# ami-iit/hippopt

Hardware: NVIDIA B200
Metric: knot_evals_per_s (higher is better)
Workload: dtype f64

## Files before the change

### hippopt_b200/_capi.py

```python
from __future__ import annotations

import ctypes
import os
import re

_HERE = os.path.dirname(os.path.abspath(__file__))
HEADER = os.path.join(os.path.dirname(_HERE), "include", "hippopt_b200.h")
LIB_PATH = os.environ.get("HIPPOPT_B200_LIB", os.path.join(_HERE, "libhippopt_b200.so"))


def parse_header(path: str = HEADER) -> dict[str, int]:
    text = open(path).read()
    text = re.sub(r"/\*.*?\*/", "", text, flags=re.S)
    text = re.sub(r"//[^\n]*", "", text)
    env: dict[str, int] = {}
    pattern = re.compile(r"#define\s+(\w+)\s+([^\n]+)|enum\s*\{([^}]*)\}", re.S)
    for mt in pattern.finditer(text):
        if mt.group(1):
            name, expr = mt.group(1), mt.group(2).strip()
            if not expr or name.endswith("_H"):
                continue
            try:
                env[name] = int(eval(expr, {"__builtins__": {}}, env))
            except Exception:
# ... 43 lines not shown
    L.hb_toy_create.argtypes = [ctypes.c_int32, ctypes.c_int32, ctypes.c_double, ctypes.POINTER(vp)]
    L.hb_destroy.restype = ctypes.c_int
    L.hb_destroy.argtypes = [vp]
    L.hb_dims.restype = ctypes.c_int
    L.hb_dims.argtypes = [vp, i64p, i64p, i64p, i64p, i64p]
    L.hb_pattern_jac.restype = ctypes.c_int
    L.hb_pattern_jac.argtypes = [vp, i64p, i64p]
    L.hb_pattern_hess.restype = ctypes.c_int
    L.hb_pattern_hess.argtypes = [vp, i64p, i64p]
    L.hb_eval.restype = ctypes.c_int
    L.hb_eval.argtypes = [vp, ctypes.c_uint32, vp, vp, ctypes.c_int64, vp, vp, vp, vp, vp, vp, vp, ctypes.c_int64, vp]
    L.hb_kino_attach_tables.restype = ctypes.c_int
    L.hb_kino_attach_tables.argtypes = [vp, i64p, i64p, i64p, i64p, i32p, f64p, i32p, f64p]
    L.hb_bounds.restype = ctypes.c_int
    L.hb_bounds.argtypes = [vp, f64p, f64p, f64p]
    L.hb_save.restype = ctypes.c_int
    L.hb_save.argtypes = [vp, ctypes.c_char_p]
    L.hb_load.restype = ctypes.c_int
    L.hb_load.argtypes = [ctypes.c_char_p, ctypes.POINTER(vp)]
    L.hb_ccs_group_mul.restype = ctypes.c_int
    L.hb_ccs_group_mul.argtypes = [vp, vp, vp, vp, vp, vp, vp, i64, i64, i64, i64, vp]
    L.hb_kkt_assemble_stage.restype = ctypes.c_int
    L.hb_kkt_assemble_stage.argtypes = [i32p, vp, vp, i64, vp, i64, vp, i64, vp, ctypes.c_double, vp, i64, vp, i64, vp, vp,
                                        vp, i64, vp]
    L.hb_external_bind.restype = ctypes.c_int
    L.hb_external_bind.argtypes = [vp]
    L.hb_external_stats.restype = ctypes.c_int
    L.hb_external_stats.argtypes = [i64p, i64p]
    L.hb_eval_cost_terms.restype = ctypes.c_int
    L.hb_eval_cost_terms.argtypes = [vp, vp, vp, ctypes.c_int64, vp, ctypes.c_int64, vp]
    L.hb_debug_sweep_schedule.restype = ctypes.c_int
    L.hb_debug_sweep_schedule.argtypes = [ctypes.c_int32, i32p, ctypes.c_int32, ctypes.c_int32, ctypes.c_int32,
                                          ctypes.c_int32, i32p, i32p]
    L.hb_host_set_parameters.restype = ctypes.c_int
    L.hb_host_set_parameters.argtypes = [vp, vp, ctypes.c_int64, ctypes.c_int64]
    L.hb_eval_host.restype = ctypes.c_int
    L.hb_eval_host.argtypes = [vp, ctypes.c_uint32, vp, vp, vp, vp, vp, vp, vp, vp, ctypes.c_int64]
    L.hb_host_last_traffic.restype = ctypes.c_int
    L.hb_host_last_traffic.argtypes = [vp, i64p, i64p]
    L.hb_host_alloc.restype = ctypes.c_int
    L.hb_host_alloc.argtypes = [ctypes.POINTER(vp), ctypes.c_int64]
    L.hb_host_free.restype = ctypes.c_int
    L.hb_host_free.argtypes = [vp]
    L.hb_lu_factor_batched.restype = ctypes.c_int
    L.hb_lu_factor_batched.argtypes = [vp, vp, vp, ctypes.c_int64, ctypes.c_int64, vp]
    L.hb_lu_solve_batched.restype = ctypes.c_int
    L.hb_lu_solve_batched.argtypes = [vp, vp, vp, ctypes.c_int64, ctypes.c_int64, ctypes.c_int64, vp]
    i64 = ctypes.c_int64
    L.hb_interpolate_humanoid_states.restype = ctypes.c_int
    L.hb_interpolate_humanoid_states.argtypes = [i64, i64, i64, vp, vp, vp, vp, i64, i64, vp, i64, i64, vp, vp, i64, i64, vp]
    L.hb_last_launch_count.restype = ctypes.c_int
    L.hb_last_launch_count.argtypes = [vp]
    L.hb_set_option.restype = ctypes.c_int
    L.hb_set_option.argtypes = [vp, ctypes.c_int32, ctypes.c_int32]
    L.hb_last_error.restype = ctypes.c_char_p
    L.hb_last_error.argtypes = []
    L.hb_profile_enable.restype = ctypes.c_int
    L.hb_profile_enable.argtypes = [vp, ctypes.c_int]
    L.hb_profile_read.restype = ctypes.c_int
    L.hb_profile_read.argtypes = [vp, f64p, i64p]
    L.hb_probe_fp64_tflops.restype = ctypes.c_int
    L.hb_probe_fp64_tflops.argtypes = [f64p, vp]
    _lib = L
    return L


EXPORTED_SYMBOLS = [
    "hb_kino_create", "hb_toy_create", "hb_destroy", "hb_dims", "hb_pattern_jac", "hb_pattern_hess", "hb_eval",
    "hb_last_launch_count", "hb_last_error", "hb_probe_fp64_tflops", "hb_profile_enable", "hb_profile_read",
    "hb_host_set_parameters", "hb_eval_host", "hb_host_last_traffic", "hb_host_alloc", "hb_host_free",
    "hb_lu_factor_batched", "hb_lu_solve_batched", "hb_set_option", "hb_interpolate_humanoid_states",
    "hb_eval_cost_terms", "hb_debug_sweep_schedule", "hb_kino_attach_tables", "hb_bounds", "hb_save", "hb_load",
    "hb_ccs_group_mul", "hb_external_bind", "hb_external_stats", "hb_kkt_assemble_stage",
] + ['hb_nlp_f', 'hb_nlp_f_n_in', 'hb_nlp_f_n_out', 'hb_nlp_f_sparsity_in', 'hb_nlp_f_sparsity_out', 'hb_nlp_f_work', 'hb_nlp_f_name_in', 'hb_nlp_f_name_out', 'hb_nlp_f_incref', 'hb_nlp_f_decref', 'hb_nlp_f_alloc_mem', 'hb_nlp_f_init_mem', 'hb_nlp_f_free_mem', 'hb_nlp_f_checkout', 'hb_nlp_f_release', 'hb_nlp_g', 'hb_nlp_g_n_in', 'hb_nlp_g_n_out', 'hb_nlp_g_sparsity_in', 'hb_nlp_g_sparsity_out', 'hb_nlp_g_work', 'hb_nlp_g_name_in', 'hb_nlp_g_name_out', 'hb_nlp_g_incref', 'hb_nlp_g_decref', 'hb_nlp_g_alloc_mem', 'hb_nlp_g_init_mem', 'hb_nlp_g_free_mem', 'hb_nlp_g_checkout', 'hb_nlp_g_release', 'hb_nlp_grad_f', 'hb_nlp_grad_f_n_in', 'hb_nlp_grad_f_n_out', 'hb_nlp_grad_f_sparsity_in', 'hb_nlp_grad_f_sparsity_out', 'hb_nlp_grad_f_work', 'hb_nlp_grad_f_name_in', 'hb_nlp_grad_f_name_out', 'hb_nlp_grad_f_incref', 'hb_nlp_grad_f_decref', 'hb_nlp_grad_f_alloc_mem', 'hb_nlp_grad_f_init_mem', 'hb_nlp_grad_f_free_mem', 'hb_nlp_grad_f_checkout', 'hb_nlp_grad_f_release', 'hb_nlp_jac_g', 'hb_nlp_jac_g_n_in', 'hb_nlp_jac_g_n_out', 'hb_nlp_jac_g_sparsity_in', 'hb_nlp_jac_g_sparsity_out', 'hb_nlp_jac_g_work', 'hb_nlp_jac_g_name_in', 'hb_nlp_jac_g_name_out', 'hb_nlp_jac_g_incref', 'hb_nlp_jac_g_decref', 'hb_nlp_jac_g_alloc_mem', 'hb_nlp_jac_g_init_mem', 'hb_nlp_jac_g_free_mem', 'hb_nlp_jac_g_checkout', 'hb_nlp_jac_g_release', 'hb_nlp_hess_l', 'hb_nlp_hess_l_n_in', 'hb_nlp_hess_l_n_out', 'hb_nlp_hess_l_sparsity_in', 'hb_nlp_hess_l_sparsity_out', 'hb_nlp_hess_l_work', 'hb_nlp_hess_l_name_in', 'hb_nlp_hess_l_name_out', 'hb_nlp_hess_l_incref', 'hb_nlp_hess_l_decref', 'hb_nlp_hess_l_alloc_mem', 'hb_nlp_hess_l_init_mem', 'hb_nlp_hess_l_free_mem', 'hb_nlp_hess_l_checkout', 'hb_nlp_hess_l_release']


class EvaluationError(RuntimeError):
    pass


def check(rc: int, what: str) -> None:
    if rc != 0:
        raise EvaluationError(f"{what} failed with code {rc}: {lib().hb_last_error().decode()}")
```

### hippopt_b200/csrc/api.cu

```cuda
#include <algorithm>
#include <cstdint>
#include <cstdio>
#include <cstring>
#include <map>
#include <string>
#include <vector>

#include "kino_const.cuh"
#include "contact_jac_desc.h"


static thread_local std::string g_err;
static int fail(int code, const std::string& msg) {
  g_err = msg;
  return code;
}
#define CUDA_TRY(expr)                                                                      \
  do {                                                                                      \
    cudaError_t e__ = (expr);                                                               \
    if (e__ != cudaSuccess) return fail(HB_ERR_CUDA, std::string(#expr) + ": " + cudaGetErrorString(e__)); \
  } while (0)

enum { KIND_KINO = 1, KIND_TOY = 2 };

// ... 78 lines not shown
  if ((e = cudaFuncSetAttribute(hb::lu_factor_kernel<3, 1>, cudaFuncAttributeMaxDynamicSharedMemorySize, lu_big)) != cudaSuccess) return e;
  if ((e = cudaFuncSetAttribute(hb::lu_factor_kernel<1, 2>, cudaFuncAttributeMaxDynamicSharedMemorySize, lu_big)) != cudaSuccess) return e;
  if ((e = cudaFuncSetAttribute(hb::lu_factor_kernel<2, 2>, cudaFuncAttributeMaxDynamicSharedMemorySize, lu_big)) != cudaSuccess) return e;
  if ((e = cudaFuncSetAttribute(hb::lu_solve_kernel, cudaFuncAttributeMaxDynamicSharedMemorySize, lu_big)) != cudaSuccess) return e;
  const int lu_staged = 232448 - 1024 - 2560;
  if ((e = cudaFuncSetAttribute(hb::lu_solve_staged_kernel<4>, cudaFuncAttributeMaxDynamicSharedMemorySize, lu_staged)) != cudaSuccess) return e;
  if ((e = cudaFuncSetAttribute(hb::lu_solve_staged_kernel<3>, cudaFuncAttributeMaxDynamicSharedMemorySize, lu_staged)) != cudaSuccess) return e;
  if ((e = cudaFuncSetAttribute(hb::lu_solve_staged_kernel<2>, cudaFuncAttributeMaxDynamicSharedMemorySize, lu_staged)) != cudaSuccess) return e;
  if ((e = cudaFuncSetAttribute(hb::lu_solve_staged_kernel<1>, cudaFuncAttributeMaxDynamicSharedMemorySize, lu_staged)) != cudaSuccess) return e;
  if ((e = cudaDeviceGetAttribute(&device_sms[dev], cudaDevAttrMultiProcessorCount, dev)) != cudaSuccess) return e;
  done[dev] = true;
  return cudaSuccess;
}

__global__ void reduce_f_kernel(const double* __restrict__ fpart, double* __restrict__ f, int n_terms, long batch) {
  const long b = (long)blockIdx.x * blockDim.x + threadIdx.x;
  if (b >= batch) return;
  const double* fp = fpart + b * n_terms;
  double acc = 0.0;
  for (int i = 0; i < n_terms; ++i) acc += fp[i];
  f[b] = acc;
}

static hb::SweepTopo sweep_topo_of(const hb::KinoConst& C) {
  hb::SweepTopo T;
  T.nb = C.nb;
  for (int l = 0; l < 32; ++l) {
    T.parent[l] = l < C.nb ? C.body[l].parent : -1;
    T.sub_mask[l] = C.sub_mask[l];
  }
  T.foot_body[0] = C.foot_body[0];
  T.foot_body[1] = C.foot_body[1];
  T.chest_body = C.chest_body;
  return T;
}

extern "C" int hb_debug_sweep_schedule(int32_t nb, const int32_t* parent, int32_t foot_l, int32_t foot_r, int32_t chest,
                                       int32_t typed, int32_t* tasks, int32_t* info) {
  if (!parent || !tasks || !info || nb < 2 || nb > 28) return fail(HB_ERR_INVALID, "hb_debug_sweep_schedule: bad argument");
  hb::SweepTopo T;
  T.nb = nb;
  for (int l = 0; l < 32; ++l) {
    T.parent[l] = l < nb ? parent[l] : -1;
    T.sub_mask[l] = 0u;
  }
  for (int l = 0; l < nb; ++l)
    for (int b = l; b >= 0; b = T.parent[b]) T.sub_mask[b] |= 1u << l;
  T.foot_body[0] = foot_l;
  T.foot_body[1] = foot_r;
  T.chest_body = chest;
  const hb::SweepSchedule s = hb::build_sweep_schedule(T, typed != 0, typed >= 2 ? 0 : 1);
  if (s.n_rounds <= 0) return fail(HB_ERR_UNSUPPORTED, "hb_debug_sweep_schedule: no schedule");
  for (size_t i = 0; i < s.tasks.size() && i < 32 * 32; ++i) tasks[i] = s.tasks[i];
  info[0] = s.n_rounds;
  info[1] = s.n_slots;
  info[2] = s.n_tasks;
  info[3] = s.n_heavy_tasks;
  info[4] = (int32_t)s.heavy_mask;
  info[5] = (int32_t)s.seed_mask;
  for (int d = 0; d < 27 && d < 4 + nb - 1; ++d) info[6 + d] = s.root_slot[d];
  return HB_OK;
}

template <class T>
static cudaError_t upload(T** dst, const T* src, size_t n) {
  cudaError_t e = cudaMalloc(dst, n * sizeof(T) + 16);
  if (e != cudaSuccess) return e;
  return cudaMemcpy(*dst, src, n * sizeof(T), cudaMemcpyHostToDevice);
}

extern "C" int hb_kino_create(const int32_t* icfg, const double* dcfg, const int32_t* jc_map, const int32_t* jk_map,
                              const int16_t* hc_index, const int32_t* hc_map, const int32_t* hk_map,
                              const int32_t* hk2_map, hb_handle* out) {
  if (!icfg || !dcfg || !jc_map || !jk_map || !hc_index || !hc_map || !hk_map || !hk2_map || !out)
    return fail(HB_ERR_INVALID, "hb_kino_create: null argument");
  hb_problem_s* h = new hb_problem_s();
  h->kind = KIND_KINO;
  cudaGetDevice(&h->device);
  hb::KinoConst& C = h->host;
  C.N = icfg[HB_KI_HORIZON];
  C.n_x = icfg[HB_KI_N_X];
  C.n_p = icfg[HB_KI_N_P];
  C.m = icfg[HB_KI_M];
  C.nnz_j = icfg[HB_KI_NNZ_J];
  C.nnz_h = icfg[HB_KI_NNZ_H];
  C.n_jc = icfg[HB_KI_N_JC];
  C.n_jk = icfg[HB_KI_N_JK];
  C.n_hc = icfg[HB_KI_N_HC];
  C.terrain = icfg[HB_KI_TERRAIN];
  C.has_final = icfg[HB_KI_HAS_FINAL];
  C.has_per = icfg[HB_KI_HAS_PERIODICITY];
  C.h_init = icfg[HB_KI_H_INIT];
  C.po_desc0 = icfg[HB_KI_PO_DESC0];
  C.po_mass = icfg[HB_KI_PO_MASS];
// ... 1354 lines not shown
```

### hippopt_b200/csrc/kino_kin.cu

```cuda
#include "kino_const.cuh"

namespace hb {

enum {
  SB_O = 0, SB_D = 3, SB_W = 6, SB_V = 9, SB_AX = 12, SB_I = 15, SB_R = 21, SB_L = 30, SB_IH = 33, SB_RHO = 36,
  SB_ACC = 39, SB_STRIDE = 51,
  SB_CB = SB_R, SB_CDB = SB_R + 3
};
enum { HSTAGE = 27 * 57 };
#ifndef HB_KIN_STAGE
#define HB_KIN_STAGE 1
#endif
#ifndef HB_KIN_STAGE_F
#define HB_KIN_STAGE_F 0
#endif
#ifndef HB_FWD_JAC
#define HB_FWD_JAC 1
#endif
#if HB_FWD_JAC && !HB_KIN_STAGE
#error "HB_FWD_JAC stages the Jacobian columns: it needs HB_KIN_STAGE"
#endif
#ifndef KIN_SCAT
#define KIN_SCAT 17
#endif
// ... 371 lines not shown
    emit.joint_t(l, dot(tax, np) + dot(ax, cn), dot(tax, wp) + dot(ax, cw));
    const int p = C.parent[l];
    const D3 rho = ld3(bl + SB_RHO), wpar = ld3(sb + p * SB_STRIDE + SB_W);
    const double inp = ((dir.mask >> p) & 1u) ? 1.0 : 0.0;
    const D3 ap = scale(inp, dir.alpha);
    const D3 trho = cross(ap, rho);
    const D3 twpar = cross(ap, wpar - dir.wpi) + scale(inp, dir.u);
    const double sd = zs[Z_SD + l - 1];
    const D3 pn = cn + cross(trho, Fp) + cross(rho, cF) + scale(sd, cross(tax, wp) + cross(ax, cw)) +
                  cross(trho, cross(vp, wpar)) + cross(rho, cross(cv, wpar) + cross(vp, twpar));
    const D3 pw = cw + cross(trho, vp) + cross(rho, cv);
    if (p == l - 1) {
      cn = pn;
      cw = pw;
    } else if (p == 0) {
      An = An + pn;
      AF = AF + cF;
      Aw = Aw + pw;
      Av = Av + cv;
    } else {
      double* sl = slot + C.slot[p] * 12 * 32 + lane;
      slot_add(sl, 0, pn);
      slot_add(sl, 3, cF);
      slot_add(sl, 6, pw);
      slot_add(sl, 9, cv);
    }
  }
  n0 = cn;
  w0 = cw;
  v0 = cv;
}

struct DirData {
  D3 alpha, pi, wpi, vpi, u;
};
__device__ __forceinline__ D3 shfl3(const D3& v, int src) {
  return v3<double>(__shfl_sync(0xffffffffu, v.x, src), __shfl_sync(0xffffffffu, v.y, src),
                    __shfl_sync(0xffffffffu, v.z, src));
}

__device__ __forceinline__ void kin_tangent_sweep_packed(const KinTopo& T, const double* sb, const double* zs,
                                                         const double* qdat, const double* massv, const SeedsT& ownS,
                                                         D3 hb, double* pslot, double* stage) {
  const int lane = threadIdx.x & 31;
  const D3 zero = v3<double>(0.0, 0.0, 0.0);
  for (int i = lane; i < T.n_pslots * 12; i += 32) pslot[i] = 0.0;
  __syncwarp();
  D3 cn = zero, cF = zero, cw = zero, cv = zero;
  unsigned t_next = (unsigned)T.sched[lane];
  for (int r = 0; r < T.n_rounds; ++r) {
    const unsigned t = t_next;
    if (r + 1 < T.n_rounds) t_next = (unsigned)T.sched[(r + 1) * 32 + lane];
    const bool valid = (t & KT_VALID) != 0;
    const int l = (t >> KT_L_SHIFT) & 31, p = (t >> KT_P_SHIFT) & 31, d = (t >> KT_D_SHIFT) & 31;
    const int src = valid ? d : lane;
    const bool heavy = (T.round_heavy_mask >> r) & 1u;
    SeedsT S;
    S.footF[0] = S.footF[1] = S.footN[0] = S.footN[1] = S.chestN = zero;
    if ((T.round_seed_mask >> r) & 1u) {
      S.footF[0] = shfl3(ownS.footF[0], src);
      S.footF[1] = shfl3(ownS.footF[1], src);
      S.footN[0] = shfl3(ownS.footN[0], src);
      S.footN[1] = shfl3(ownS.footN[1], src);
      S.chestN = shfl3(ownS.chestN, src);
    }
    if (valid) {
      if (t & KT_START) cn = cF = cw = cv = zero;
      const double* bl = sb + l * SB_STRIDE;
      const D3 ax = ld3(bl + SB_AX);
      D3 tax = zero, trho = zero, twpar = zero;
      const D3 rho = ld3(bl + SB_RHO), wpar = ld3(sb + p * SB_STRIDE + SB_W);
      if (heavy) {
        DirData dir;
        {
          const double* bd = sb + (d < 4 ? 0 : d - 3) * SB_STRIDE;
          dir.wpi = ld3(bd + SB_W);
          dir.vpi = ld3(bd + SB_V);
          if (d < 4) {
            dir.alpha = ld3(qdat + 6 * d);
            dir.u = ld3(qdat + 6 * d + 3);
            dir.pi = zero;
          } else {
            dir.alpha = ld3(bd + SB_AX);
            dir.u = zero;
            dir.pi = ld3(bd + SB_O);
          }
        }
        const double m = massv[l];
        const bool in = (t & KT_IN_L) != 0;
        const D3 a = in ? dir.alpha : zero, uu = in ? dir.u : zero;
        const D3 d_ = ld3(bl + SB_D), w = ld3(bl + SB_W);
        const D3 rr = ld3(bl + SB_O) - dir.pi;
        const D3 to = cross(a, rr);
        const D3 td = cross(a, d_);
        const D3 tw = cadd(uu, a, w - dir.wpi);
        const D3 tv = cadd(cadd(cross(dir.wpi, to), a, (ld3(bl + SB_V) - dir.vpi) - cross(dir.wpi, rr)), uu, rr);
        tax = cross(a, ax);
        if (in) {
          const double* I = bl + SB_I;
          const D3 cbar = ld3(bl + SB_CB), cdbar = ld3(bl + SB_CDB), Ih = ld3(bl + SB_IH), Iw = ld3(bl + SB_L);
          const D3 tc = to + td;
          const D3 tcd = cadd(cadd(tv, tw, d_), w, td);
          const D3 tcbar = scale(m, cross(tcd, hb));
          const D3 tcdbar = scale(m, cross(hb, tc));
          const D3 tIw = cadd(symmul(I, tw - cross(a, w)), a, Iw);
          const D3 tIh = csub(cross(a, Ih), I, cross(a, hb));
          cF = cF + tcbar;
          D3 n1 = cadd(cadd(cadd(cn, td, cbar), d_, tcbar), td, cross(cdbar, w));
          D3 n2 = cadd(cadd(cadd(cross(d_, cadd(cross(tcdbar, w), cdbar, tw)), tIw, hb), tIh, w), Ih, tw);
          cn = n1 + n2;
          cv = cv + tcdbar;
          cw = cadd(cadd(cw, td, cdbar), d_, tcdbar) + tIh;
        }
        if (t & KT_IN_P) {
          trho = cross(dir.alpha, rho);
          twpar = cadd(dir.u, dir.alpha, wpar - dir.wpi);
        }
      }
      if (l == T.foot_body[0]) {
        cF = cF + S.footF[0];
        cn = cn + S.footN[0];
      }
      if (l == T.foot_body[1]) {
        cF = cF + S.footF[1];
        cn = cn + S.footN[1];
      }
      if (l == T.chest_body) cn = cn + S.chestN;
      const int ls = (t >> KT_LOAD_SHIFT) & 63;
      if (ls) {
        const double* sl = pslot + (ls - 1) * 12;
        cn = cn + ld3(sl);
        cF = cF + ld3(sl + 3);
        cw = cw + ld3(sl + 6);
        cv = cv + ld3(sl + 9);
      }
      if (l != 0) {
        double* col = stage + d * 57;
        const double sd = zs[Z_SD + l - 1];
        if (heavy) {
          const D3 np = ld3(bl + SB_ACC), Fp = ld3(bl + SB_ACC + 3), wp = ld3(bl + SB_ACC + 6), vp = ld3(bl + SB_ACC + 9);
          col[7 + l - 1] += dot(tax, wp) + dot(ax, cw);
          col[34 + l - 1] += dot(tax, np) + dot(ax, cn);
          D3 n1 = cadd(cadd(cn, trho, Fp), rho, cF);
          D3 n2 = cadd(scale(sd, cadd(cross(tax, wp), ax, cw)), trho, cross(vp, wpar));
          cn = cadd(n1 + n2, rho, cadd(cross(cv, wpar), vp, twpar));
          cw = cadd(cadd(cw, trho, vp), rho, cv);
        } else {
          col[7 + l - 1] += dot(ax, cw);
          col[34 + l - 1] += dot(ax, cn);
// ... 574 lines not shown
        unsigned w[8];
#pragma unroll
        for (int u = 0; u < 8; ++u) w[u] = (eb + 32 * u) < n ? lst[eb + 32 * u] : 0xffffffffu;
#pragma unroll
        for (int u = 0; u < 8; ++u)
          if (w[u] != 0xffffffffu) em.jac[w[u] & 0xffffu] = st[w[u] >> 16];
      }
      __syncwarp();
    }
    if (want_grad) {
      double* gf = grad_f + b * T.n_x + (long)k * T.x_stride;
      for (int i = lane; i < 57; i += 32) {
        int off;
        if (i < 3) off = Z_VB + i;
        else if (i < 7) off = Z_QD + i - 3;
        else if (i < 11) off = Z_Q + i - 7;
        else if (i < 34) off = Z_SD + i - 11;
        else off = Z_S + i - 34;
        if (C.zmap[off] >= 0) gf[C.zmap[off]] = gbuf[i];
      }
      if (lane < 3 && C.zmap[Z_PB + lane] >= 0) gf[C.zmap[Z_PB + lane]] = 0.0;
    }
  }
  if (!WITH_HESS) return;
  if (!with_l && !(HB_FWD_JAC && (want_jac || want_grad))) return;
  {
    const int dirj = lane < 27 ? lane : -1;
    Dir dir;
    dir.mask = 0u;
    dir.alpha = dir.pi = dir.wpi = dir.vpi = dir.u = v3<double>(0.0, 0.0, 0.0);
    double* qdat = zs;
    double* qw = zs + 48;
    double* qK = zs + 60;
    static_assert(48 + 12 + 32 <= Z_VB && HB_N_JOINTS + 1 <= 24, "quaternion tables overlap z or the masses");
    if (lane < 4) {
      D3 g, u, w;
      const double qraw[4] = {q0, q1, q2, q3};
      quat_map<double>(qraw, qdv, lane, g, u, w);
      st3(qdat + 6 * lane, g);
      st3(qdat + 6 * lane + 3, u);
      st3(qw + 3 * lane, w);
    }
    __syncwarp();
    D3 wq_lane = v3<double>(0.0, 0.0, 0.0);
    if (lane >= 3 && lane < 7) wq_lane = ld3(qw + 3 * (lane - 3));
    if (lane < 4) {
      dir.alpha = ld3(qdat + 6 * lane);
      dir.u = ld3(qdat + 6 * lane + 3);
      dir.mask = 0xffffffffu;
      dir.wpi = ld3(sb + SB_W);
      dir.vpi = ld3(sb + SB_V);
    } else if (lane < 27) {
      const int l = lane - 4 + 1;
      dir.mask = C.sub_mask[l];
      const double* bl = sb + l * SB_STRIDE;
      dir.alpha = ld3(bl + SB_AX);
      dir.pi = ld3(bl + SB_O);
      dir.wpi = ld3(bl + SB_W);
      dir.vpi = ld3(bl + SB_V);
    }
    enum { CM_M = 0, CM_P = 1, CM_PD = 4, CM_H = 7, CM_J = 10, CM_STRIDE = 17 };
    double* comp = sm + L.stage;
    if (lane < nb) {
      const double* bl = sb + lane * SB_STRIDE;
      const double m = my_mass;
      const D3 c = ld3(bl + SB_O) + ld3(bl + SB_D);
      const D3 cd = ld3(bl + SB_V) + cross(ld3(bl + SB_W), ld3(bl + SB_D));
// ... 43 lines not shown
    }
    HB_PHASE(0, 4);
    D3 tP, tPd, th;
    {
      const double* cm = comp + (lane >= 4 && lane < 27 ? lane - 3 : 0) * CM_STRIDE;
      const double Ms = cm[CM_M];
      const D3 P = ld3(cm + CM_P), Pds = ld3(cm + CM_PD), Hs = ld3(cm + CM_H);
      const D3 a = dir.alpha, beta = cross(dir.alpha, dir.wpi);
      const D3 Pr = P - scale(Ms, dir.pi);
      tP = cross(a, Pr);
      tPd = cross(a, Pds - scale(Ms, dir.vpi)) - cross(beta, Pr) + cross(dir.u, P);
      th = cross(a, Hs) - cross(cross(a, dir.pi), Pds) - cross(P, cross(a, dir.vpi)) - symmul(cm + CM_J, beta) +
           cross(P, cross(beta, dir.pi)) + symmul(cm + CM_J, dir.u);
    }
    D3 vel_dh = v3<double>(0.0, 0.0, 0.0);
    D3 vel_pv = vel_dh;
    if (lane < 30) {
      D3 A = v3<double>(0.0, 0.0, 0.0), B = A, piv = A;
      int lv = 0;
      if (lane < 3) B = v3<double>(lane == 0 ? 1.0 : 0.0, lane == 1 ? 1.0 : 0.0, lane == 2 ? 1.0 : 0.0);
      else if (lane < 7) A = wq_lane;
      else {
        lv = lane - 6;
        A = ld3(sb + lv * SB_STRIDE + SB_AX);
        piv = ld3(sb + lv * SB_STRIDE + SB_O);
      }
      const double* cm = comp + lv * CM_STRIDE;
      const double Ms = cm[CM_M];
      const D3 P = ld3(cm + CM_P);
      const D3 pv = cross(A, P - scale(Ms, piv)) + scale(Ms, B);
      const D3 hv = symmul(cm + CM_J, A) - cross(P, cross(A, piv)) + cross(P, B);
      vel_dh = scale(-1.0 / mass_p, hv - scale(1.0 / M, cross(Pm, pv)));
      vel_pv = pv;
    }
    __syncwarp();
    const V3<Dual> xcD = lift<Dual>(xc, scale(1.0 / M, tP));
    const V3<Dual> xdD = lift<Dual>(xcd, scale(1.0 / M, tPd));
    const double inL = ((dir.mask >> T.foot_body[0]) & 1u) ? 1.0 : 0.0;
    const double inR = ((dir.mask >> T.foot_body[1]) & 1u) ? 1.0 : 0.0;
    const double inC = ((dir.mask >> T.chest_body) & 1u) ? 1.0 : 0.0;
    double ty_lane, tphi_lane;
    {
      const D3 a = dir.alpha;
      const D3 tL = scale(inL, cross(a, (ld3(sb + T.foot_body[0] * SB_STRIDE + SB_O) - dir.pi) + fdal));
      const D3 tR = scale(inR, cross(a, (ld3(sb + T.foot_body[1] * SB_STRIDE + SB_O) - dir.pi) + fdar));
      ty_lane = dot(scale(inR, cross(a, fdu)), fdDelta) + dot(fdu, tL - tR);
      const D3 ac = scale(inC, a);
      tphi_lane = cross(ac, v3<double>(G[0], G[3], G[6])).x + cross(ac, v3<double>(G[1], G[4], G[7])).y +
                  cross(ac, v3<double>(G[2], G[5], G[8])).z;
    }
    HB_PHASE(0, 5);
#if HB_FWD_JAC
    if (want_jac || want_grad) {
      double* stg = sm + L.stage;
      const int bm = 4 + 648 + 81;
      if (want_jac) {
        if (lane < 27) {
#pragma unroll
          for (int pt = 0; pt < 8; ++pt) {
            const int f = pt >> 2;
            const double in = f == 0 ? inL : inR;
            const D3 r = (ld3(sb + T.foot_body[f] * SB_STRIDE + SB_O) - dir.pi) + ld3(sm + L.arms + 3 * pt);
            const D3 t = scale(-in, cross(dir.alpha, r));
            stg[4 + (3 * pt) * 27 + lane] = t.x;
            stg[4 + (3 * pt + 1) * 27 + lane] = t.y;
            stg[4 + (3 * pt + 2) * 27 + lane] = t.z;
// ... 98 lines not shown
      S.footF[1] = S.footF[1] - ku;
      S.footN[1] = S.footN[1] + scale(kd, cross(uD, dD)) - cross(arD, ku);
    }
    {
      const D3 a = scale(inC, dir.alpha);
      double tG[9];
#pragma unroll
      for (int j = 0; j < 3; ++j) {
        const D3 col = v3<double>(G[j], G[3 + j], G[6 + j]);
        const D3 t = cross(a, col);
        tG[j] = t.x;
        tG[3 + j] = t.y;
        tG[6 + j] = t.z;
      }
      const double tphi = tG[0] + tG[4] + tG[8];
      const double cw = k1 ? 2.0 * sg * T.w_frame : 0.0;
      const Dual kappa = mkdual(cw * (phi - 3.0), cw * tphi);
      const V3<Dual> mGD = lift<Dual>(mG, v3<double>(tG[5] - tG[7], tG[6] - tG[2], tG[1] - tG[3]));
      S.chestN = scale(kappa, mGD);
    }
    HessEmit em;
    em.map = C.hk_map + T.knot_maps[k].hk_off;
    em.hess = hess + b * T.nnz_h + T.knot_maps[k].hk_base;
    em.stage = HB_KIN_STAGE ? sm + L.stage : nullptr;
    em.dirj = dirj;
    em.add_sd = em.add_s = 0.0;
    if (lane >= 4 && lane < 27 && k1) {
      const double wjl = C.wj[lane - 4];
      em.add_sd = T.joint_cost_kind == 0 ? sg * T.w_joint * 2.0 * wjl : 0.0;
      em.add_s = T.joint_cost_kind == 0 ? sg * T.w_joint * 2.0 * wjl * wjl : sg * T.w_joint * 2.0 * wjl;
    }
    V3<Dual> n0, w0, v0;
    const double lu_pre = lamk[31];
#ifdef HB_DUAL_SWEEP
    kin_backward<Dual>(T, sb, zs, dir, S, xcD, xdD, slot, em, n0, w0, v0);
#else
    {
      SeedsP SP;
      SeedsT ST;
      SP.wc = S.wc;
      SP.hb = S.hb;
#pragma unroll
      for (int f = 0; f < 2; ++f) {
        SP.footF[f] = primal_of(S.footF[f]);
        SP.footN[f] = primal_of(S.footN[f]);
        ST.footF[f] = tangent_of(S.footF[f]);
        ST.footN[f] = tangent_of(S.footN[f]);
      }
      SP.chestN = primal_of(S.chestN);
      ST.chestN = tangent_of(S.chestN);
      __syncwarp();
      HB_PHASE(0, 8);
      primal_adjoint_pass(T, sb, zs, SP, xc, xcd, my_depth, my_rank, my_parent, my_mass);
      HB_PHASE(0, 9);
      D3 tn0, tw0, tv0;
#if HB_SWEEP_PACKED
      {
        double* stg = sm + L.stage;
        double* pslot = sm + L.gbuf;
        constexpr int XT = 7;
        double* xt = pslot;
        double* massv = zs + 24;
        if (lane < 27) {
          st3(xt + (30 + lane) * XT, tP);
          st3(xt + (30 + lane) * XT + 3, tPd);
        }
        if (lane < 30) st3(xt + lane * XT + 3, vel_pv);
        if (lane < nb) massv[lane] = my_mass;
        __syncwarp();
        if (lane < 27) {
          const D3 hbv = S.hb;
          const D3 a1 = cross(tPd, hbv), a2 = cross(hbv, tP);
          double* col = stg + lane * 57;
          const double sM = -1.0 / M;
#pragma unroll 5
          for (int r = 0; r < 30; ++r) col[r] = sM * dot(ld3(xt + XT * r + 3), a2);
#pragma unroll 2
          for (int j = 0; j < 14; ++j) {
            const int e = lane + j < 27 ? lane + j : lane + j - 27;
            const double* xe = xt + XT * (30 + e);
            const double v = sM * (dot(ld3(xe), a1) + dot(ld3(xe + 3), a2));
            col[30 + e] = v;
            stg[e * 57 + 30 + lane] = v;
          }
          if (lane >= 4) {
            col[7 + lane - 4] += em.add_sd;
            col[34 + lane - 4] += em.add_s;
          }
        }
        __syncwarp();
        HB_PHASE(0, 10);
        em.acc = true;
        kin_tangent_sweep_packed(T, sb, zs, qdat, massv, ST, S.hb, pslot, stg);
        HB_PHASE(0, 11);
        const double* rs = pslot + (lane < 27 ? T.root_slot[lane] : 0) * 12;
        tn0 = ld3(rs);
        tw0 = ld3(rs + 6);
        tv0 = ld3(rs + 9);
      }
#else
      kin_tangent_sweep(T, sb, zs, dir, S.hb, ST, tangent_of(xcD), tangent_of(xdD), slot, em, tn0, tw0, tv0);
#endif
      n0 = lift<Dual>(ld3(sb + SB_ACC), tn0);
      w0 = lift<Dual>(ld3(sb + SB_ACC + 6), tw0);
      v0 = lift<Dual>(ld3(sb + SB_ACC + 9), tv0);
    }
#endif
    if (lane < 16) {
      const int a = lane >> 2, bq = lane & 3;
      Dual qD[4];
      double qdv2[4];
#pragma unroll
      for (int i = 0; i < 4; ++i) {
        qD[i] = mkdual(zs[Z_Q + i], i == bq ? 1.0 : 0.0);
        qdv2[i] = zs[Z_QD + i];
      }
      V3<Dual> g, u, w;
      quat_map<Dual>(qD, qdv2, a, g, u, w);
      const D3 pn0 = primal_of(n0), pw0 = primal_of(w0);
      qK[lane] = dot(pn0, tangent_of(g)) + dot(pw0, tangent_of(u));
      qK[16 + lane] = dot(pw0, tangent_of(w));
    }
    __syncwarp();
    if (dirj >= 0) {
      const D3 tn0 = tangent_of(n0), tw0 = tangent_of(w0);
      em.put(0, v0.x.d);
      em.put(1, v0.y.d);
      em.put(2, v0.z.d);
      const double lu = lu_pre;
      const double nqd = rbq[0] * rbq[0] + rbq[1] * rbq[1] + rbq[2] * rbq[2] +
                         rbq[3] * rbq[3];
#pragma unroll
      for (int a = 0; a < 4; ++a) {
        const bool qdir = lane < 4;
        const double dq = dot(tn0, ld3(qdat + 6 * a)) + dot(tw0, ld3(qdat + 6 * a + 3)) + (qdir ? qK[4 * a + lane] : 0.0);
        const double dqd = dot(tw0, ld3(qw + 3 * a)) + (qdir ? qK[16 + 4 * a + lane] : 0.0);
        const double extra = (a == lane && k1) ? 2.0 * sg * T.w_bq * nqd + 2.0 * lu : 0.0;
        em.put(3 + a, dqd);
        em.put(30 + a, dq + extra);
      }
    }
    HB_PHASE(0, 12);
    __syncwarp();
    if (em.stage) {
      const double* st = sm + L.stage;
#if HB_KIN_HESS_LIST
      const int2 hkl = *reinterpret_cast<const int2*>(&T.knot_maps[k].hk_off);
      const unsigned* lst = C.hk_list + hkl.x;
      const int n = hkl.y;
      for (int eb = lane; eb < n; eb += 32 * KIN_SCAT) {
        unsigned w[KIN_SCAT];
#pragma unroll
        for (int u = 0; u < KIN_SCAT; ++u) w[u] = (eb + 32 * u) < n ? lst[eb + 32 * u] : 0xffffffffu;
#pragma unroll
        for (int u = 0; u < KIN_SCAT; ++u)
          if (w[u] != 0xffffffffu) em.hess[w[u] & 0xffffu] = st[w[u] >> 16];
      }
#else
      for (int eb = lane; eb < HSTAGE; eb += 32 * KIN_SCAT) {
        int sl[KIN_SCAT];
#pragma unroll
        for (int u = 0; u < KIN_SCAT; ++u) sl[u] = (eb + 32 * u) < HSTAGE ? em.map[eb + 32 * u] : -1;
#pragma unroll
        for (int u = 0; u < KIN_SCAT; ++u)
          if (sl[u] >= 0) em.hess[sl[u]] = st[eb + 32 * u];
      }
#endif
    }
    if (lane < 27) {
      const int2 hk2m = *reinterpret_cast<const int2*>(&T.knot_maps[k].hk2_base);
      const int slot2 = C.hk2_map[hk2m.y + lane];
      if (slot2 >= 0)
// ... 15 lines not shown
```

### hippopt_b200/csrc/sweep_schedule.h

```cpp
#pragma once
#include <algorithm>
#include <map>
#include <utility>
#include <vector>

namespace hb {

enum {
  KT_L_SHIFT = 0, KT_P_SHIFT = 5, KT_D_SHIFT = 10, KT_VALID = 1 << 15, KT_START = 1 << 16, KT_IN_L = 1 << 17,
  KT_IN_P = 1 << 18, KT_LOAD_SHIFT = 19, KT_FLUSH_SHIFT = 25, KT_STORE = 1u << 31
};

struct SweepTopo {
  int nb = 0;
  int parent[32];
  int foot_body[2];
  int chest_body = 0;
  unsigned sub_mask[32];
};

struct SweepSchedule {
  std::vector<int> tasks;
  int n_rounds = 0, n_slots = 0, n_tasks = 0, n_heavy_tasks = 0;
  unsigned seed_mask = 0;
  unsigned heavy_mask = 0;
  int root_slot[32] = {0};
};

inline SweepSchedule build_sweep_schedule(const SweepTopo& C, bool typed_rounds = true, int policy = 1) {
  const int nb = C.nb, n_dir = 4 + (nb - 1);
  struct Seg {
    int d;
    std::vector<int> bodies;
    int flush_body;
    int crit = 0, lane = -1, next = 0, flushed = -1;
    std::vector<int> round_of;
  };
  std::vector<Seg> segs;
  std::vector<std::vector<int>> slot_of(n_dir, std::vector<int>(nb, -1));
  std::vector<std::vector<char>> in_full(n_dir, std::vector<char>(nb, 0));
  int n_slots = 0;
  for (int d = 0; d < n_dir; ++d) {
    const int ld = d < 4 ? 0 : d - 3;
    std::vector<char> rel(nb, 0);
    for (int l = 0; l < nb; ++l)
      if ((C.sub_mask[ld] >> l) & 1u) in_full[d][l] = rel[l] = 1;
    for (int a = C.parent[ld]; a >= 0; a = C.parent[a]) rel[a] = 1;
    for (int f = 0; f < 2; ++f)
      if (in_full[d][C.foot_body[f]])
        for (int a = C.foot_body[1 - f]; a >= 0; a = C.parent[a]) rel[a] = 1;
    std::vector<int> height(nb, 0), main_child(nb, -1);
    for (int l = nb - 1; l >= 1; --l) {
      if (!rel[l]) continue;
      const int p = C.parent[l];
      if (rel[p] && height[l] + 1 > height[p]) {
        height[p] = height[l] + 1;
        main_child[p] = l;
      }
    }
    slot_of[d][0] = n_slots++;
    for (int l = nb - 1; l >= 1; --l) {
      if (!rel[l]) continue;
      bool leaf = true;
      for (int c = l + 1; c < nb; ++c)
        if (rel[c] && C.parent[c] == l) leaf = false;
      if (!leaf) continue;
      Seg s;
      s.d = d;
      int b = l;
      for (;;) {
        s.bodies.push_back(b);
        const int p = C.parent[b];
        if (p == 0 || main_child[p] != b) {
          s.flush_body = p;
          break;
// ... 148 lines not shown
```

### include/hippopt_b200.h

```cpp
#ifndef HIPPOPT_B200_H
#define HIPPOPT_B200_H

#include <stdint.h>

#ifdef __cplusplus
extern "C" {
#endif

typedef struct hb_problem_s* hb_handle;

enum {
  HB_EVAL_F = 1,
  HB_EVAL_GRAD_F = 2,
  HB_EVAL_G = 4,
  HB_EVAL_JAC_G = 8,
  HB_EVAL_HESS_L = 16
};

enum { HB_OK = 0, HB_ERR_INVALID = 1, HB_ERR_CUDA = 2, HB_ERR_UNSUPPORTED = 3 };

#define HB_MAX_BODIES 32
#define HB_N_JOINTS 23
#define HB_N_POINTS 8

// ... 245 lines not shown
int hb_nlp_jac_g(const double** arg, double** res, hb_casadi_int* iw, double* w, int mem);
hb_casadi_int hb_nlp_jac_g_n_in(void);
hb_casadi_int hb_nlp_jac_g_n_out(void);
const hb_casadi_int* hb_nlp_jac_g_sparsity_in(hb_casadi_int i);
const hb_casadi_int* hb_nlp_jac_g_sparsity_out(hb_casadi_int i);
int hb_nlp_jac_g_work(hb_casadi_int* sz_arg, hb_casadi_int* sz_res, hb_casadi_int* sz_iw, hb_casadi_int* sz_w);
const char* hb_nlp_jac_g_name_in(hb_casadi_int i);
const char* hb_nlp_jac_g_name_out(hb_casadi_int i);
void hb_nlp_jac_g_incref(void);
void hb_nlp_jac_g_decref(void);
int hb_nlp_jac_g_alloc_mem(void);
int hb_nlp_jac_g_init_mem(int mem);
void hb_nlp_jac_g_free_mem(int mem);
int hb_nlp_jac_g_checkout(void);
void hb_nlp_jac_g_release(int mem);
int hb_nlp_hess_l(const double** arg, double** res, hb_casadi_int* iw, double* w, int mem);
hb_casadi_int hb_nlp_hess_l_n_in(void);
hb_casadi_int hb_nlp_hess_l_n_out(void);
const hb_casadi_int* hb_nlp_hess_l_sparsity_in(hb_casadi_int i);
const hb_casadi_int* hb_nlp_hess_l_sparsity_out(hb_casadi_int i);
int hb_nlp_hess_l_work(hb_casadi_int* sz_arg, hb_casadi_int* sz_res, hb_casadi_int* sz_iw, hb_casadi_int* sz_w);
const char* hb_nlp_hess_l_name_in(hb_casadi_int i);
const char* hb_nlp_hess_l_name_out(hb_casadi_int i);
void hb_nlp_hess_l_incref(void);
void hb_nlp_hess_l_decref(void);
int hb_nlp_hess_l_alloc_mem(void);
int hb_nlp_hess_l_init_mem(int mem);
void hb_nlp_hess_l_free_mem(int mem);
int hb_nlp_hess_l_checkout(void);
void hb_nlp_hess_l_release(int mem);

int hb_debug_sweep_schedule(int32_t nb, const int32_t* parent, int32_t foot_l, int32_t foot_r, int32_t chest,
                            int32_t typed, int32_t* tasks, int32_t* info);

const char* hb_last_error(void);

int hb_probe_fp64_tflops(double* tflops, void* stream);

#ifdef __cplusplus
}
#endif
#endif
```

Measured before the change: 22.70 million.

## Compute base-orientation tangent directions in closed form instead of through the packed sweep

Removes the four base-quaternion directions from the packed tangent sweep schedule (n_base=0 in the device topology) and computes their root tangent contributions analytically in lanes 0-3, storing them in a new shared table. Stage columns are patched to add the missing terms via lam_al and vel_dh rows. This shortens the sweep schedule (fewer tasks and rounds) at the cost of extra closed-form arithmetic and more complex correctness reasoning. The debug schedule API gains an n_base variant that keeps the old default of 4.

```diff
diff --git a/hippopt_b200/_capi.py b/hippopt_b200/_capi.py
--- a/hippopt_b200/_capi.py
+++ b/hippopt_b200/_capi.py
@@ -99,6 +99,9 @@
     L.hb_debug_sweep_schedule.restype = ctypes.c_int
     L.hb_debug_sweep_schedule.argtypes = [ctypes.c_int32, i32p, ctypes.c_int32, ctypes.c_int32, ctypes.c_int32,
                                           ctypes.c_int32, i32p, i32p]
+    L.hb_debug_sweep_schedule_n_base.restype = ctypes.c_int
+    L.hb_debug_sweep_schedule_n_base.argtypes = [ctypes.c_int32, i32p, ctypes.c_int32, ctypes.c_int32, ctypes.c_int32,
+                                                 ctypes.c_int32, ctypes.c_int32, i32p, i32p]
     L.hb_host_set_parameters.restype = ctypes.c_int
     L.hb_host_set_parameters.argtypes = [vp, vp, ctypes.c_int64, ctypes.c_int64]
     L.hb_eval_host.restype = ctypes.c_int
@@ -137,7 +140,8 @@
     "hb_last_launch_count", "hb_last_error", "hb_probe_fp64_tflops", "hb_profile_enable", "hb_profile_read",
     "hb_host_set_parameters", "hb_eval_host", "hb_host_last_traffic", "hb_host_alloc", "hb_host_free",
     "hb_lu_factor_batched", "hb_lu_solve_batched", "hb_set_option", "hb_interpolate_humanoid_states",
-    "hb_eval_cost_terms", "hb_debug_sweep_schedule", "hb_kino_attach_tables", "hb_bounds", "hb_save", "hb_load",
+    "hb_eval_cost_terms", "hb_debug_sweep_schedule", "hb_debug_sweep_schedule_n_base", "hb_kino_attach_tables",
+    "hb_bounds", "hb_save", "hb_load",
     "hb_ccs_group_mul", "hb_external_bind", "hb_external_stats", "hb_kkt_assemble_stage",
 ] + ['hb_nlp_f', 'hb_nlp_f_n_in', 'hb_nlp_f_n_out', 'hb_nlp_f_sparsity_in', 'hb_nlp_f_sparsity_out', 'hb_nlp_f_work', 'hb_nlp_f_name_in', 'hb_nlp_f_name_out', 'hb_nlp_f_incref', 'hb_nlp_f_decref', 'hb_nlp_f_alloc_mem', 'hb_nlp_f_init_mem', 'hb_nlp_f_free_mem', 'hb_nlp_f_checkout', 'hb_nlp_f_release', 'hb_nlp_g', 'hb_nlp_g_n_in', 'hb_nlp_g_n_out', 'hb_nlp_g_sparsity_in', 'hb_nlp_g_sparsity_out', 'hb_nlp_g_work', 'hb_nlp_g_name_in', 'hb_nlp_g_name_out', 'hb_nlp_g_incref', 'hb_nlp_g_decref', 'hb_nlp_g_alloc_mem', 'hb_nlp_g_init_mem', 'hb_nlp_g_free_mem', 'hb_nlp_g_checkout', 'hb_nlp_g_release', 'hb_nlp_grad_f', 'hb_nlp_grad_f_n_in', 'hb_nlp_grad_f_n_out', 'hb_nlp_grad_f_sparsity_in', 'hb_nlp_grad_f_sparsity_out', 'hb_nlp_grad_f_work', 'hb_nlp_grad_f_name_in', 'hb_nlp_grad_f_name_out', 'hb_nlp_grad_f_incref', 'hb_nlp_grad_f_decref', 'hb_nlp_grad_f_alloc_mem', 'hb_nlp_grad_f_init_mem', 'hb_nlp_grad_f_free_mem', 'hb_nlp_grad_f_checkout', 'hb_nlp_grad_f_release', 'hb_nlp_jac_g', 'hb_nlp_jac_g_n_in', 'hb_nlp_jac_g_n_out', 'hb_nlp_jac_g_sparsity_in', 'hb_nlp_jac_g_sparsity_out', 'hb_nlp_jac_g_work', 'hb_nlp_jac_g_name_in', 'hb_nlp_jac_g_name_out', 'hb_nlp_jac_g_incref', 'hb_nlp_jac_g_decref', 'hb_nlp_jac_g_alloc_mem', 'hb_nlp_jac_g_init_mem', 'hb_nlp_jac_g_free_mem', 'hb_nlp_jac_g_checkout', 'hb_nlp_jac_g_release', 'hb_nlp_hess_l', 'hb_nlp_hess_l_n_in', 'hb_nlp_hess_l_n_out', 'hb_nlp_hess_l_sparsity_in', 'hb_nlp_hess_l_sparsity_out', 'hb_nlp_hess_l_work', 'hb_nlp_hess_l_name_in', 'hb_nlp_hess_l_name_out', 'hb_nlp_hess_l_incref', 'hb_nlp_hess_l_decref', 'hb_nlp_hess_l_alloc_mem', 'hb_nlp_hess_l_init_mem', 'hb_nlp_hess_l_free_mem', 'hb_nlp_hess_l_checkout', 'hb_nlp_hess_l_release']
 
diff --git a/hippopt_b200/csrc/api.cu b/hippopt_b200/csrc/api.cu
--- a/hippopt_b200/csrc/api.cu
+++ b/hippopt_b200/csrc/api.cu
@@ -134,14 +134,18 @@
   T.foot_body[0] = C.foot_body[0];
   T.foot_body[1] = C.foot_body[1];
   T.chest_body = C.chest_body;
+  T.n_base = 0;
   return T;
 }
 
-extern "C" int hb_debug_sweep_schedule(int32_t nb, const int32_t* parent, int32_t foot_l, int32_t foot_r, int32_t chest,
-                                       int32_t typed, int32_t* tasks, int32_t* info) {
-  if (!parent || !tasks || !info || nb < 2 || nb > 28) return fail(HB_ERR_INVALID, "hb_debug_sweep_schedule: bad argument");
+extern "C" int hb_debug_sweep_schedule_n_base(int32_t nb, const int32_t* parent, int32_t foot_l, int32_t foot_r,
+                                              int32_t chest, int32_t typed, int32_t n_base, int32_t* tasks,
+                                              int32_t* info) {
+  if (!parent || !tasks || !info || nb < 2 || nb > 28 || n_base < 0 || n_base > 4)
+    return fail(HB_ERR_INVALID, "hb_debug_sweep_schedule: bad argument");
   hb::SweepTopo T;
   T.nb = nb;
+  T.n_base = n_base;
   for (int l = 0; l < 32; ++l) {
     T.parent[l] = l < nb ? parent[l] : -1;
     T.sub_mask[l] = 0u;
@@ -162,6 +166,11 @@
   info[5] = (int32_t)s.seed_mask;
   for (int d = 0; d < 27 && d < 4 + nb - 1; ++d) info[6 + d] = s.root_slot[d];
   return HB_OK;
+}
+
+extern "C" int hb_debug_sweep_schedule(int32_t nb, const int32_t* parent, int32_t foot_l, int32_t foot_r, int32_t chest,
+                                       int32_t typed, int32_t* tasks, int32_t* info) {
+  return hb_debug_sweep_schedule_n_base(nb, parent, foot_l, foot_r, chest, typed, 4, tasks, info);
 }
 
 template <class T>
diff --git a/hippopt_b200/csrc/kino_kin.cu b/hippopt_b200/csrc/kino_kin.cu
--- a/hippopt_b200/csrc/kino_kin.cu
+++ b/hippopt_b200/csrc/kino_kin.cu
@@ -427,7 +427,7 @@
 }
 
 struct DirData {
-  D3 alpha, pi, wpi, vpi, u;
+  D3 alpha, pi, wpi, vpi;
 };
 __device__ __forceinline__ D3 shfl3(const D3& v, int src) {
   return v3<double>(__shfl_sync(0xffffffffu, v.x, src), __shfl_sync(0xffffffffu, v.y, src),
@@ -435,8 +435,8 @@
 }
 
 __device__ __forceinline__ void kin_tangent_sweep_packed(const KinTopo& T, const double* sb, const double* zs,
-                                                         const double* qdat, const double* massv, const SeedsT& ownS,
-                                                         D3 hb, double* pslot, double* stage) {
+                                                         const double* massv, const SeedsT& ownS, D3 hb, double* pslot,
+                                                         double* stage) {
   const int lane = threadIdx.x & 31;
   const D3 zero = v3<double>(0.0, 0.0, 0.0);
   for (int i = lane; i < T.n_pslots * 12; i += 32) pslot[i] = 0.0;
@@ -468,28 +468,21 @@
       if (heavy) {
         DirData dir;
         {
-          const double* bd = sb + (d < 4 ? 0 : d - 3) * SB_STRIDE;
+          const double* bd = sb + (d - 3) * SB_STRIDE;
           dir.wpi = ld3(bd + SB_W);
           dir.vpi = ld3(bd + SB_V);
-          if (d < 4) {
-            dir.alpha = ld3(qdat + 6 * d);
-            dir.u = ld3(qdat + 6 * d + 3);
-            dir.pi = zero;
-          } else {
-            dir.alpha = ld3(bd + SB_AX);
-            dir.u = zero;
-            dir.pi = ld3(bd + SB_O);
-          }
+          dir.alpha = ld3(bd + SB_AX);
+          dir.pi = ld3(bd + SB_O);
         }
         const double m = massv[l];
         const bool in = (t & KT_IN_L) != 0;
-        const D3 a = in ? dir.alpha : zero, uu = in ? dir.u : zero;
+        const D3 a = in ? dir.alpha : zero;
         const D3 d_ = ld3(bl + SB_D), w = ld3(bl + SB_W);
         const D3 rr = ld3(bl + SB_O) - dir.pi;
         const D3 to = cross(a, rr);
         const D3 td = cross(a, d_);
-        const D3 tw = cadd(uu, a, w - dir.wpi);
-        const D3 tv = cadd(cadd(cross(dir.wpi, to), a, (ld3(bl + SB_V) - dir.vpi) - cross(dir.wpi, rr)), uu, rr);
+        const D3 tw = cross(a, w - dir.wpi);
+        const D3 tv = cadd(cross(dir.wpi, to), a, (ld3(bl + SB_V) - dir.vpi) - cross(dir.wpi, rr));
         tax = cross(a, ax);
         if (in) {
           const double* I = bl + SB_I;
@@ -509,7 +502,7 @@
         }
         if (t & KT_IN_P) {
           trho = cross(dir.alpha, rho);
-          twpar = cadd(dir.u, dir.alpha, wpar - dir.wpi);
+          twpar = cross(dir.alpha, wpar - dir.wpi);
         }
       }
       if (l == T.foot_body[0]) {
@@ -1150,7 +1143,8 @@
     double* qdat = zs;
     double* qw = zs + 48;
     double* qK = zs + 60;
-    static_assert(48 + 12 + 32 <= Z_VB && HB_N_JOINTS + 1 <= 24, "quaternion tables overlap z or the masses");
+    double* qt = zs + 92;
+    static_assert(92 + 24 <= Z_VB && HB_N_JOINTS + 1 <= 24, "quaternion tables overlap z or the masses");
     if (lane < 4) {
       D3 g, u, w;
       const double qraw[4] = {q0, q1, q2, q3};
@@ -1260,6 +1254,34 @@
       const D3 hv = symmul(cm + CM_J, A) - cross(P, cross(A, piv)) + cross(P, B);
       vel_dh = scale(-1.0 / mass_p, hv - scale(1.0 / M, cross(Pm, pv)));
       vel_pv = pv;
+    }
+    if (with_l) {
+      double* Tm = qK;
+      if (lane < 9) {
+        const int i = lane / 3, j = lane % 3;
+        double t = -(i == 0 ? xc.x : (i == 1 ? xc.y : xc.z)) * lamk[24 + j];
+#pragma unroll
+        for (int pt = 0; pt < 8; ++pt)
+          t -= (sb[T.foot_body[pt >> 2] * SB_STRIDE + SB_O + i] + sm[L.arms + 3 * pt + i]) * lamk[3 * pt + j];
+        Tm[lane] = t;
+      }
+      __syncwarp();
+      if (lane < 4) {
+        const D3 a = dir.alpha, om = ld3(sb + SB_W), hbv = scale(-1.0 / mass_p, ld3(lamk + 27));
+        const double* J0 = comp + CM_J;
+        const D3 ah = cross(a, hbv);
+        const D3 w0 = symmul(J0, hbv) - scale(1.0 / M, cross(Pm, cross(hbv, Pm)));
+        const D3 tw0 = cross(a, w0) - (symmul(J0, ah) - scale(1.0 / M, cross(Pm, cross(ah, Pm))));
+        const D3 dhang = th - scale(1.0 / M, cross(tP, Pd) + cross(Pm, tPd));
+        const double trT = Tm[0] + Tm[4] + Tm[8];
+        const double cf = k1 ? 2.0 * sg * T.w_frame : 0.0, kap = cf * (phi - 3.0);
+        D3 tn0 = v3<double>(Tm[0] * a.x + Tm[1] * a.y + Tm[2] * a.z, Tm[3] * a.x + Tm[4] * a.y + Tm[5] * a.z,
+                            Tm[6] * a.x + Tm[7] * a.y + Tm[8] * a.z) - scale(trT, a);
+        tn0 = tn0 + cross(dhang, hbv) - cross(dir.u, w0) - cross(om, tw0);
+        tn0 = tn0 + scale(cf * dot(a, mG), mG) + scale(kap, matvec(G, a) - scale(phi, a));
+        st3(qt + 6 * lane, tn0);
+        st3(qt + 6 * lane + 3, tw0);
+      }
     }
     __syncwarp();
     const V3<Dual> xcD = lift<Dual>(xc, scale(1.0 / M, tP));
@@ -1424,6 +1446,7 @@
     }
     V3<Dual> n0, w0, v0;
     const double lu_pre = lamk[31];
+    const D3 lam_al = cross(ld3(lamk + 27), dir.alpha);
 #ifdef HB_DUAL_SWEEP
     kin_backward<Dual>(T, sb, zs, dir, S, xcD, xdD, slot, em, n0, w0, v0);
 #else
@@ -1457,7 +1480,10 @@
           st3(xt + (30 + lane) * XT, tP);
           st3(xt + (30 + lane) * XT + 3, tPd);
         }
-        if (lane < 30) st3(xt + lane * XT + 3, vel_pv);
+        if (lane < 30) {
+          st3(xt + lane * XT, vel_dh);
+          st3(xt + lane * XT + 3, vel_pv);
+        }
         if (lane < nb) massv[lane] = my_mass;
         __syncwarp();
         if (lane < 27) {
@@ -1465,8 +1491,12 @@
           const D3 a1 = cross(tPd, hbv), a2 = cross(hbv, tP);
           double* col = stg + lane * 57;
           const double sM = -1.0 / M;
+          const bool qc = lane < 4;
+          const D3 cr = qc ? lam_al : a2;
+          const double sc = qc ? 1.0 : sM;
+          const double* xr0 = xt + (qc ? 0 : 3);
 #pragma unroll 5
-          for (int r = 0; r < 30; ++r) col[r] = sM * dot(ld3(xt + XT * r + 3), a2);
+          for (int r = 0; r < 30; ++r) col[r] = sc * dot(ld3(xr0 + XT * r), cr);
 #pragma unroll 2
           for (int j = 0; j < 14; ++j) {
             const int e = lane + j < 27 ? lane + j : lane + j - 27;
@@ -1483,12 +1513,19 @@
         __syncwarp();
         HB_PHASE(0, 10);
         em.acc = true;
-        kin_tangent_sweep_packed(T, sb, zs, qdat, massv, ST, S.hb, pslot, stg);
+        kin_tangent_sweep_packed(T, sb, zs, massv, ST, S.hb, pslot, stg);
         HB_PHASE(0, 11);
-        const double* rs = pslot + (lane < 27 ? T.root_slot[lane] : 0) * 12;
-        tn0 = ld3(rs);
-        tw0 = ld3(rs + 6);
-        tv0 = ld3(rs + 9);
+        if (lane < 4) {
+          tn0 = ld3(qt + 6 * lane);
+          tw0 = ld3(qt + 6 * lane + 3);
+          tv0 = v3<double>(0.0, 0.0, 0.0);
+        } else {
+          const double* rs = pslot + (lane < 27 ? T.root_slot[lane] : 0) * 12;
+          tn0 = ld3(rs);
+          tw0 = ld3(rs + 6);
+          tv0 = ld3(rs + 9);
+        }
+        em.acc = lane >= 4;
       }
 #else
       kin_tangent_sweep(T, sb, zs, dir, S.hb, ST, tangent_of(xcD), tangent_of(xdD), slot, em, tn0, tw0, tv0);
@@ -1530,6 +1567,9 @@
         const double extra = (a == lane && k1) ? 2.0 * sg * T.w_bq * nqd + 2.0 * lu : 0.0;
         em.put(3 + a, dqd);
         em.put(30 + a, dq + extra);
+#if HB_SWEEP_PACKED && !defined(HB_DUAL_SWEEP)
+        if (lane >= 4) em.stage[a * 57 + 34 + lane - 4] += dq;
+#endif
       }
     }
     HB_PHASE(0, 12);
diff --git a/hippopt_b200/csrc/sweep_schedule.h b/hippopt_b200/csrc/sweep_schedule.h
--- a/hippopt_b200/csrc/sweep_schedule.h
+++ b/hippopt_b200/csrc/sweep_schedule.h
@@ -17,6 +17,7 @@
   int foot_body[2];
   int chest_body = 0;
   unsigned sub_mask[32];
+  int n_base = 4;
 };
 
 struct SweepSchedule {
@@ -41,6 +42,7 @@
   std::vector<std::vector<char>> in_full(n_dir, std::vector<char>(nb, 0));
   int n_slots = 0;
   for (int d = 0; d < n_dir; ++d) {
+    if (d < 4 && d >= C.n_base) continue;
     const int ld = d < 4 ? 0 : d - 3;
     std::vector<char> rel(nb, 0);
     for (int l = 0; l < nb; ++l)
diff --git a/include/hippopt_b200.h b/include/hippopt_b200.h
--- a/include/hippopt_b200.h
+++ b/include/hippopt_b200.h
@@ -301,6 +301,8 @@
 
 int hb_debug_sweep_schedule(int32_t nb, const int32_t* parent, int32_t foot_l, int32_t foot_r, int32_t chest,
                             int32_t typed, int32_t* tasks, int32_t* info);
+int hb_debug_sweep_schedule_n_base(int32_t nb, const int32_t* parent, int32_t foot_l, int32_t foot_r, int32_t chest,
+                                   int32_t typed, int32_t n_base, int32_t* tasks, int32_t* info);
 
 const char* hb_last_error(void);
 
```

Measured after the change: 23.94 million, median of 6. +5.5%, better.
